# Gadersd/whisper-burn

Hardware: NVIDIA H100
Metric: audio-seconds/sec (higher is better)
Workload: dtype f32 (fp16-exact weights, fp32 activations/accumulate)

## Files before the change

whisper-burn_b200/csrc/api.cu:

```cuda
#include <algorithm>
#include <cstring>
#include <map>
#include <memory>
#include <mutex>
#include <new>

#include "../host/beam.hpp"
#include "../host/repeat.hpp"
#include "session.h"

struct wb_model {
    wb::Model impl;
    std::mutex fwd_mu;
    std::unique_ptr<wb::Session> fwd;
    wb::Session& forward_session(int64_t n_windows, int64_t text_len) {
        if (!fwd || fwd->max_windows < n_windows || fwd->t_max < text_len) {
            fwd.reset();
            fwd.reset(new wb::Session(&impl, std::max<int64_t>(n_windows, 1), 1, std::max<int64_t>(text_len, 2), WB_KV_F32));
        }
        return *fwd;
    }
    ~wb_model() { fwd.reset(); }
};
struct wb_session {
// ... 351 lines not shown
        if (!S.encoded) wb::fail(WB_ERR_STATE, "get_mel: nothing encoded");
        WB_REQUIRE(window >= 0 && window < S.n_windows, "get_mel: window out of range");
        const int Tm = S.win_Tm[(size_t)window];
        WB_REQUIRE(capacity >= (int64_t)Tm * wb::N_MELS, "get_mel: capacity too small");
        std::vector<float> rows((size_t)Tm * wb::N_MELS);
        WB_CUDA(cudaMemcpy(rows.data(), S.mel_rows.p + ((int64_t)window * S.TmS + 1) * wb::N_MELS,
                           rows.size() * sizeof(float), cudaMemcpyDeviceToHost));
        for (int t = 0; t < Tm; ++t)
            for (int c = 0; c < wb::N_MELS; ++c) mel_out[(int64_t)c * Tm + t] = rows[(size_t)t * wb::N_MELS + c];
        *n_ctx_out = Tm;
    });
}

int wb_session_get_encoder_output(wb_session* s, int64_t window, float* out, int64_t capacity, int64_t* n_ctx_out) {
    return guarded([&] {
        WB_REQUIRE(s && out && n_ctx_out, "get_encoder_output: null pointer");
        wb::Session& S = *s->impl;
        if (!S.encoded) wb::fail(WB_ERR_STATE, "get_encoder_output: nothing encoded");
        WB_REQUIRE(window >= 0 && window < S.n_windows, "get_encoder_output: window out of range");
        const int d = S.m->dims.n_audio_state;
        const int T = S.win_T[(size_t)window];
        WB_REQUIRE(capacity >= (int64_t)T * d, "get_encoder_output: capacity too small");
        WB_CUDA(cudaMemcpy(out, S.xa.p + S.win_row_off[(size_t)window] * d, (size_t)T * d * sizeof(float),
                           cudaMemcpyDeviceToHost));
        *n_ctx_out = T;
    });
}

int wb_session_begin(wb_session* s, const int64_t* prompt, int64_t prompt_len) {
    return guarded([&] {
        WB_REQUIRE(s && prompt, "begin: null pointer");
        WB_REQUIRE(prompt_len >= 1, "begin: prompt length out of range");
        s->impl->begin(std::vector<std::vector<int64_t>>((size_t)s->impl->n_windows, std::vector<int64_t>(prompt, prompt + prompt_len)));
    });
}

int wb_session_step(wb_session* s, int64_t n_rows, const int32_t* window_of_row, const int32_t* parent_row,
                    const int64_t* token, int apply_special_mask, const uint8_t* is_special, int k,
                    int64_t* topk_ids_out, float* topk_logprob_out) {
    return guarded([&] {
        WB_REQUIRE(s && window_of_row && parent_row && token && topk_ids_out && topk_logprob_out, "step: null pointer");
        if (is_special) s->impl->set_special(is_special);
        WB_REQUIRE(!apply_special_mask || s->impl->have_special, "step: special mask requested but no is_special bitmap given");
        s->impl->step_beams(n_rows, window_of_row, parent_row, token, apply_special_mask, k, topk_ids_out, topk_logprob_out);
    });
}

int wb_transcribe_windows(wb_session* s, const float* const* waves, const int64_t* lens, int64_t n_windows,
                          int beam_size, int max_depth, const wb_special_ids* ids, const uint8_t* is_special,
                          int64_t* tokens_out, int64_t capacity, int64_t* lens_out) {
    return guarded([&] {
        WB_REQUIRE(s && waves && lens && ids && tokens_out && lens_out, "transcribe: null pointer");
        wb::Session& S = *s->impl;
        const auto prompts = wb::window_prompts(S, n_windows, beam_size, max_depth, *ids, is_special);
        copy_tokens_out(wb::transcribe_windows(S, prompts, beam_size, max_depth, ids->eot, is_special, capacity,
                                               [&] { S.encode_waveforms_host(waves, lens, n_windows); }),
                        tokens_out, capacity, lens_out);
    });
}

int wb_transcribe_windows_prev(wb_session* s, const float* const* waves, const int64_t* lens, int64_t n_windows,
                               const int64_t* prev_tokens, const int64_t* prev_lens, int64_t startofprev, int beam_size,
                               int max_depth, const wb_special_ids* ids, const uint8_t* is_special, int64_t* tokens_out,
                               int64_t capacity, int64_t* lens_out) {
    return guarded([&] {
        WB_REQUIRE(s && waves && lens && prev_lens && ids && tokens_out && lens_out, "transcribe_windows_prev: null pointer");
// ... 263 lines not shown
```

whisper-burn_b200/csrc/session.cu:

```cuda
#include <algorithm>
#include <cmath>
#include <cstdio>
#include <cstdlib>
#include <cstring>

#include "session.h"

namespace wb {

int window_mel_frames(int n_audio_ctx, int window_mode) {
    WB_REQUIRE(window_mode == WB_WINDOWS_REFERENCE || window_mode == WB_WINDOWS_NATIVE,
               "window_mode must be WB_WINDOWS_REFERENCE or WB_WINDOWS_NATIVE");
    return window_mode == WB_WINDOWS_NATIVE ? 2 * n_audio_ctx : n_audio_ctx;
}

int64_t window_samples(int n_audio_ctx, int window_mode) {
    return wb_max_waveform_samples(window_mel_frames(n_audio_ctx, window_mode) - MEL_PADDING);
}

Session::Session(Model* model, int64_t max_w, int64_t max_b, int64_t max_text_len, int kv, int mode) : m(model) {
    if (!m || !m->finalized) fail(WB_ERR_STATE, "session: model not finalized");
    const wb_dims& D = m->dims;
    WB_REQUIRE(max_w >= 1 && max_b >= 1 && max_w * max_b <= 4096, "session: bad max_windows / max_beams");
    WB_REQUIRE(max_text_len >= 2 && max_text_len <= D.n_text_ctx, "session: max_text_len must be in [2, n_text_ctx]");
// ... 54 lines not shown
    is_special.alloc(V);
    {
        ckv_tmp.alloc(Mcap * 2 * d);
        cudaDeviceProp prop;
        WB_CUDA(cudaGetDeviceProperties(&prop, m->device));
        n_sm = prop.multiProcessorCount;
        const int n_logit_ctas = 2 * prop.multiProcessorCount;
        part_o.alloc((size_t)Rmax * H * 16 * 64); part_m.alloc((size_t)Rmax * H * 16); part_l.alloc((size_t)Rmax * H * 16);
        datt.alloc((size_t)Rmax * d); steps_done.alloc(128); dec_bar.alloc(4);
        WB_CUDA(cudaMemsetAsync(dec_bar.p, 0, 4 * sizeof(unsigned int), st));
        {
            const bool h16 = m->fp16_exact;
            auto wp = [&](const LinearW& w) -> const void* { return h16 ? (const void*)w.w16 : (const void*)w.w32; };
            std::vector<DecLayer> lay((size_t)L);
            for (int l = 0; l < L; ++l) {
                const DecBlockW& B = m->dec[(size_t)l];
                DecLayer& y = lay[(size_t)l];
                y.ln1_g = B.attn_ln.g; y.ln1_b = B.attn_ln.b; y.ln1_eps = B.attn_ln.eps;
                y.ln2_g = B.cross_ln.g; y.ln2_b = B.cross_ln.b; y.ln2_eps = B.cross_ln.eps;
                y.ln3_g = B.mlp_ln.g; y.ln3_b = B.mlp_ln.b; y.ln3_eps = B.mlp_ln.eps;
                y.Wqkv = wp(B.qkv); y.Wo = wp(B.out); y.Wcq = wp(B.cq); y.Wco = wp(B.cout); y.W1 = wp(B.mlp1); y.W2 = wp(B.mlp2);
                y.bqkv = B.qkv.b; y.bo = B.out.b; y.bcq = B.cq.b; y.bco = B.cout.b; y.b1 = B.mlp1.b; y.b2 = B.mlp2.b;
            }
            dec_layers.alloc((size_t)L);
            WB_CUDA(cudaMemcpy(dec_layers.p, lay.data(), lay.size() * sizeof(DecLayer), cudaMemcpyHostToDevice));
        }
        dec5_build_tables(*m, n_sm, d5);
        ypart.alloc((size_t)4 * Rmax * d);
        lg_m.alloc((size_t)n_logit_ctas * Rmax); lg_s.alloc((size_t)n_logit_ctas * Rmax);
        lg_v.alloc((size_t)n_logit_ctas * Rmax * DEC_KC); lg_i.alloc((size_t)n_logit_ctas * Rmax * DEC_KC);
    }
    h_parent = pinned<int>(Rmax); h_window = pinned<int>(Rmax); h_token = pinned<int>(Rmax);
    h_topk_id = pinned<int>((size_t)Rmax * DEC_KC);
    WB_CUDA(cudaMemsetAsync(is_special.p, 0, V, st));

    DecArgs& a = dec_base;
    a.Rmax = Rmax; a.d = D.n_text_state; a.H = H; a.L = L; a.V = V; a.t_max = t_max; a.Mcap = Mcap;
    a.eps_outside = m->ln_eps_outside; a.qk_scale = (float)std::pow((double)D.n_text_state / (double)H, -0.25);
    a.layers = dec_layers.p; a.tok_emb = m->tok_emb32; a.pos_emb = m->dec_pos;
    a.E = m->fp16_exact ? (const void*)m->tok_emb16 : (const void*)m->tok_emb32;
    a.E_tiled = m->tok_emb16_tiled;
    a.lnf_g = m->dec_ln.g; a.lnf_b = m->dec_ln.b; a.lnf_eps = m->dec_ln.eps;
    a.x = dx.p; a.q = dq.p; a.att = datt.p; a.hid = dhid.p;
    a.ypart = ypart.p; a.lgbuf = logits.p; a.att_pl = att_pl.p; a.hid_pl = hid_pl.p;
    a.kv_half = kv == WB_KV_F16 ? 1 : 0;
    if (a.kv_half) { a.kc = kc16.p; a.vc = vc16.p; a.ckv = ckv16.p; } else { a.kc = kc.p; a.vc = vc.p; a.ckv = ckv.p; }
    a.row_window = row_window.p; a.win_row_off = d_win_row_off.p; a.win_T = d_win_T.p;
    a.part_o = part_o.p; a.part_m = part_m.p; a.part_l = part_l.p;
    a.tokens = tokens.p; a.token_lp = token_lp.p; a.cur_tok = cur_tok.p; a.lengths = lengths.p; a.finished = finished.p;
    a.eot_logit = eot_logit.p; a.topk_id = topk_id.p; a.topk_lp = topk_lp.p;
    a.lg_m = lg_m.p; a.lg_s = lg_s.p; a.lg_v = lg_v.p; a.lg_i = lg_i.p;
    a.pos = pos.p; a.n_unfinished = n_unfinished.p; a.steps_done = steps_done.p; a.bar = dec_bar.p;
    WB_CUDA(cudaStreamSynchronize(st));
}

Session::~Session() {
    if (st) cudaStreamSynchronize(st);
    for (auto& e : ev)
        if (e) cudaEventDestroy(e);
    if (st) cudaStreamDestroy(st);
}

static void set_geometry(Session& s, const std::vector<int>& Tm, const std::vector<int>& F) {
    s.n_windows = (int)Tm.size();
    s.win_Tm = Tm;
    s.win_F = F;
    s.win_T.resize(Tm.size());
    s.win_row_off.resize(Tm.size());
    s.M_tot = 0;
    s.max_T = 0;
    s.max_Tm = 0;
    for (size_t w = 0; w < Tm.size(); ++w) {
        s.win_T[w] = (Tm[w] - 1) / 2 + 1;
        s.win_row_off[w] = s.M_tot;
        s.M_tot += s.win_T[w];
        s.max_T = std::max(s.max_T, s.win_T[w]);
        s.max_Tm = std::max(s.max_Tm, Tm[w]);
    }
    const int d = s.m->dims.n_audio_state;
    std::vector<GemmGroup> g1(Tm.size()), g2(Tm.size());
    std::vector<AttnWindow> aw(Tm.size());
    for (size_t w = 0; w < Tm.size(); ++w) {
        g1[w] = GemmGroup{(int64_t)w * s.TmS * N_MELS, ((int64_t)w * s.TmS + 1) * d, Tm[w]};
        g2[w] = GemmGroup{(int64_t)w * s.TmS * d, s.win_row_off[w] * d, s.win_T[w]};
        aw[w] = AttnWindow{s.win_row_off[w], s.win_T[w]};
    }
    WB_CUDA(cudaMemcpyAsync(s.d_g1.p, g1.data(), g1.size() * sizeof(GemmGroup), cudaMemcpyHostToDevice, s.st));
    WB_CUDA(cudaMemcpyAsync(s.d_g2.p, g2.data(), g2.size() * sizeof(GemmGroup), cudaMemcpyHostToDevice, s.st));
    WB_CUDA(cudaMemcpyAsync(s.d_awin.p, aw.data(), aw.size() * sizeof(AttnWindow), cudaMemcpyHostToDevice, s.st));
    WB_CUDA(cudaMemcpyAsync(s.d_win_row_off.p, s.win_row_off.data(), Tm.size() * sizeof(int64_t),
                            cudaMemcpyHostToDevice, s.st));
    WB_CUDA(cudaMemcpyAsync(s.d_win_T.p, s.win_T.data(), Tm.size() * sizeof(int), cudaMemcpyHostToDevice, s.st));
    WB_CUDA(cudaStreamSynchronize(s.st));
}

void Session::encode_from_device_wave(const float* wave_dev, const int64_t* offsets, const int64_t* lens, int64_t n) {
    WB_REQUIRE(n >= 1 && n <= max_windows, "encode: n_windows out of range for this session");
    std::vector<LogMelWindow> lw((size_t)n);
    std::vector<int> Tm((size_t)n), kept((size_t)n);
    int max_frames = 0;
    for (int64_t w = 0; w < n; ++w) {
        WB_REQUIRE(lens[w] >= N_FFT, "prep_audio: waveform shorter than n_fft (audio.rs:292)");
        WB_REQUIRE(lens[w] < (int64_t)1 << 30, "prep_audio: waveform too long");
        const int F = (int)(lens[w] / HOP);
        const int keep = std::min(F, mel_limit - MEL_PADDING);
        Tm[(size_t)w] = keep + MEL_PADDING;
        kept[(size_t)w] = keep;
        lw[(size_t)w] = LogMelWindow{offsets[w], (int)lens[w], F, keep, (int)w, ((int64_t)w * TmS + 1) * N_MELS};
        max_frames = std::max(max_frames, F);
    }
    WB_CUDA(cudaMemcpyAsync(d_lmwin.p, lw.data(), lw.size() * sizeof(LogMelWindow), cudaMemcpyHostToDevice, st));
    set_geometry(*this, Tm, kept);
    WB_CUDA(cudaEventRecord(ev[0], st));
    WB_CUDA(cudaMemsetAsync(mel_rows.p, 0, (size_t)n * TmS * N_MELS * sizeof(float), st));
    launch_logmel(*m, wave_dev, d_lmwin.p, (int)n, max_frames, mel_rows.p, max_slots.p, (int)n, st);
    WB_CUDA(cudaEventRecord(ev[1], st));
    run_encoder();
    WB_CUDA(cudaEventRecord(ev[2], st));
}

void Session::encode_waveforms_host(const float* const* waves, const int64_t* lens, int64_t n) {
    WB_REQUIRE(n >= 1 && n <= max_windows, "encode: n_windows out of range for this session");
    std::vector<int64_t> offs((size_t)n);
    int64_t total = 0;
    for (int64_t w = 0; w < n; ++w) {
        WB_REQUIRE(waves[w] != nullptr && lens[w] >= 0, "encode: null waveform");
        offs[(size_t)w] = total;
        total += (lens[w] + 3) / 4 * 4;
    }
    wave.ensure((size_t)total);
    for (int64_t w = 0; w < n; ++w)
        WB_CUDA(cudaMemcpyAsync(wave.p + offs[(size_t)w], waves[w], (size_t)lens[w] * sizeof(float),
                                cudaMemcpyHostToDevice, st));
    encode_from_device_wave(wave.p, offs.data(), lens, n);
}

void Session::encode_mels_host(const float* mel, int64_t n, int64_t n_mels, int64_t n_ctx) {
    const wb_dims& D = m->dims;
    WB_REQUIRE(n_mels == D.n_mels, "Audio mel spectrum size must be n_mels (mod.rs:231-235)");
    WB_REQUIRE(n_ctx >= 1 && n_ctx <= mel_limit, "Audio length cannot exceed the session's mel frame limit: n_audio_ctx, "
                                                 "2 * n_audio_ctx in native windowing (mod.rs:236-241)");
    WB_REQUIRE(n >= 1 && n <= max_windows, "encode: n_windows out of range for this session");
    std::vector<int> Tm((size_t)n, (int)n_ctx);
    set_geometry(*this, Tm, Tm);
    DevBuf<float> tmp;
// ... 106 lines not shown
        p = GemmParams{};
        p.A = hid.p; p.lda = 4 * d; p.B = B.mlp2.w32; p.C = x.p; p.ldc = d; p.N = d; p.K = 4 * d;
        p.bias = B.mlp2.b; p.residual = x.p; p.max_rows = M;
        launch_gemm(p, st);
    }
    launch_layernorm(x.p, xa.p, nullptr, nullptr, m->ln_post, M, d, m->ln_eps_outside, st);
}

void Session::run_cross_kv() {
    const wb_dims& D = m->dims;
    const int d = D.n_text_state;
    const float qk_scale = (float)std::pow((double)d / (double)D.n_text_head, -0.25);
    for (int l = 0; l < D.n_text_layer; ++l) {
        const DecBlockW& B = m->dec[(size_t)l];
        if (use_tc) {
            GemmF16Params p;
            p.A_hi = xa_h.p; p.A_lo = xa_l.p; p.lda = d; p.B = B.ckv.w16; p.C = ckv_tmp.p; p.ldc = 2 * d;
            p.N = 2 * d; p.K = d; p.bias = B.ckv.b; p.scale = qk_scale; p.scale_cols = d; p.max_rows = (int)M_tot;
            GemmF16Plan& pl = *enc_plans[(size_t)2 + 4 * D.n_audio_layer + l];
            if (!pl.matches(p.max_rows, 1)) pl.build(p, 0, (int)M_tot);
            pl.launch(st);
        } else {
            GemmParams p;
            p.A = xa.p; p.lda = d; p.B = B.ckv.w32; p.C = ckv_tmp.p; p.ldc = 2 * d;
            p.N = 2 * d; p.K = d; p.bias = B.ckv.b; p.scale = qk_scale; p.scale_cols = d; p.max_rows = (int)M_tot;
            launch_gemm(p, st);
        }
        void* dst = kv_dtype == WB_KV_F16 ? (void*)(ckv16.p + (size_t)l * Mcap * 2 * d) : (void*)(ckv.p + (size_t)l * Mcap * 2 * d);
        launch_ckv_relayout(ckv_tmp.p, dst, kv_dtype == WB_KV_F16, d_win_row_off.p, d_win_T.p, n_windows, M_tot, d, st);
    }
}

void Session::set_special(const uint8_t* sp) {
    if (sp) {
        WB_CUDA(cudaMemcpyAsync(is_special.p, sp, (size_t)m->dims.n_vocab, cudaMemcpyHostToDevice, st));
        WB_CUDA(cudaStreamSynchronize(st));
        have_special = true;
    }
}

void Session::seat_rows(int rows, int per_window, const std::vector<std::vector<int64_t>>& prompts, int max_depth) {
    if (!encoded) fail(WB_ERR_STATE, "session: decode before encode");
    WB_REQUIRE(rows <= Rmax && (int64_t)prompts.size() * per_window >= rows, "decode: rows out of range");
    const int V = m->dims.n_vocab;
    std::vector<int> tk((size_t)rows * t_max, 0), rw((size_t)rows), len((size_t)rows), lim((size_t)rows);
    for (int r = 0; r < rows; ++r) {
        const std::vector<int64_t>& pr = prompts[(size_t)(r / per_window)];
        WB_REQUIRE(!pr.empty() && (int64_t)pr.size() <= t_max, "decode: prompt length out of range");
        rw[(size_t)r] = r / per_window;
        len[(size_t)r] = (int)pr.size();
        lim[(size_t)r] = (int)pr.size() + max_depth;
        for (size_t i = 0; i < pr.size(); ++i) {
            WB_REQUIRE(pr[i] >= 0 && pr[i] < V, "decode: prompt token out of range");
            tk[(size_t)r * t_max + i] = (int)pr[i];
        }
    }
    WB_CUDA(cudaMemcpyAsync(tokens.p, tk.data(), tk.size() * sizeof(int), cudaMemcpyHostToDevice, st));
    WB_CUDA(cudaMemcpyAsync(row_window.p, rw.data(), rw.size() * sizeof(int), cudaMemcpyHostToDevice, st));
    WB_CUDA(cudaMemsetAsync(finished.p, 0, sizeof(int) * Rmax, st));
    WB_CUDA(cudaMemsetAsync(pos.p, 0, sizeof(int), st));
    WB_CUDA(cudaMemcpyAsync(lengths.p, len.data(), len.size() * sizeof(int), cudaMemcpyHostToDevice, st));
    WB_CUDA(cudaMemcpyAsync(lengths.p + Rmax, lim.data(), lim.size() * sizeof(int), cudaMemcpyHostToDevice, st));
    R = rows;
    anc_identity = true;
    anc_cur = 0;
    host_pos = 0;
}

void Session::feed_positions(int n, float* logits_out) {
    const size_t V = (size_t)m->dims.n_vocab;
    const StepLogits out = logits_out ? StepLogits::topk_and_raw : StepLogits::none;
    for (int p = 0; p < n; ++p, ++host_pos) {
        WB_CUDA(cudaMemcpy2DAsync(cur_tok.p, sizeof(int), tokens.p + p, t_max * sizeof(int), sizeof(int), R, cudaMemcpyDeviceToDevice, st));
        launch_decoder(DecodeLaunch::cached_step(R, host_pos, out, MASK_NONE, 1));
        if (logits_out)
            WB_CUDA(cudaMemcpy2DAsync(logits_out + p * V, n * V * sizeof(float), logits.p, V * sizeof(float), V * sizeof(float), R,
                                      cudaMemcpyDeviceToHost, st));
    }
}

static std::pair<int, int> prompt_range(const std::vector<std::vector<int64_t>>& prompts) {
    int lo = INT_MAX, hi = 0;
    for (const auto& pr : prompts) { lo = std::min(lo, (int)pr.size()); hi = std::max(hi, (int)pr.size()); }
    return {lo, hi};
}

void Session::begin(const std::vector<std::vector<int64_t>>& prompts, bool prefill, int max_depth) {
    WB_REQUIRE((int64_t)prompts.size() == n_windows, "begin: one prompt per encoded window");
    for (const auto& pr : prompts) WB_REQUIRE(!pr.empty() && (int64_t)pr.size() < t_max, "begin: prompt length out of range");
    seat_rows(n_windows, 1, prompts, max_depth);
    if (prefill) feed_positions(prompt_range(prompts).first - 1, nullptr);
    WB_CUDA(cudaStreamSynchronize(st));
}

void Session::teacher_forced_logits(const int64_t* toks, int64_t n_rows, int64_t seq_len, float* logits_out) {
    WB_REQUIRE(n_rows >= 1 && seq_len >= 1, "forward_decoder: empty input");
    std::vector<std::vector<int64_t>> rows((size_t)n_rows);
    for (int64_t r = 0; r < n_rows; ++r) rows[(size_t)r].assign(toks + r * seq_len, toks + (r + 1) * seq_len);
    seat_rows((int)n_rows, 1, rows);
    feed_positions((int)seq_len, logits_out);
    WB_CUDA(cudaStreamSynchronize(st));
}

bool Session::launch_decoder(const DecodeLaunch& l) {
    DecArgs a = dec_base;
    a.R = l.rows;
    a.lg_slices = std::max(1, std::min(16, n_sm / std::max(1, l.rows)));
    a.n_splits = std::max(1, std::min(16, n_sm / std::max(1, l.rows * a.H)));
    a.anc = anc_identity ? nullptr : (anc_cur == 0 ? anc0.p : anc1.p);
    a.use_cur_tok = l.use_cur_tok; a.pos0 = l.pos0; a.n_steps = l.n_steps; a.logits_from = l.logits_from;
    a.is_special = have_special ? is_special.p : nullptr; a.mask_mode = l.mask_mode;
    a.k = l.k; a.greedy = l.greedy; a.eot = l.eot; a.loop_rules = l.loop_rules; a.max_depth = l.max_depth;
    a.logits_out = l.raw_logits ? logits.p : nullptr;
    if (getenv("WB200_TRACE")) {
        dec_trace.ensure(1 << 16);
        WB_CUDA(cudaMemsetAsync(dec_trace.p, 0, sizeof(unsigned long long) * (1 << 16), st));
        a.trace = dec_trace.p;
        a.trace_cap = 1 << 16;
    }
    WB_CUDA(cudaMemsetAsync(dec_bar.p, 0, 4 * sizeof(unsigned int), st));
    const bool h16 = m->fp16_exact;
    auto allowed = [&](int n) { return only_decoder == 0 || only_decoder == n; };
    int groups = 0;
    last_groups = 1;
    if (l.beam > 1) {
// ... 63 lines not shown
    }
    {
        int* cur = anc_cur == 0 ? anc0.p : anc1.p;
        int* nxt = anc_cur == 0 ? anc1.p : anc0.p;
        R = (int)n_rows;
        launch_dec_reorder(cur, nxt, parent.p, pos.p, R, t_max, st);
        anc_cur ^= 1;
    }
    launch_decoder(DecodeLaunch::cached_step(R, host_pos, StepLogits::topk, apply_mask ? MASK_ALWAYS : MASK_NONE, k));
    ++host_pos;
    WB_CUDA(cudaMemcpyAsync(h_topk_id.get(), topk_id.p, sizeof(int) * n_rows * k, cudaMemcpyDeviceToHost, st));
    WB_CUDA(cudaMemcpyAsync(topk_lp_out, topk_lp.p, sizeof(float) * n_rows * k, cudaMemcpyDeviceToHost, st));
    WB_CUDA(cudaStreamSynchronize(st));
    for (int64_t i = 0; i < n_rows * k; ++i) topk_ids_out[i] = h_topk_id[i];
}

void Session::last_topk(int64_t n_rows, int64_t k, int64_t* ids_out, float* lp_out) {
    if (last_decoder == 0) fail(WB_ERR_STATE, "last_topk: no decoder launch yet");
    WB_REQUIRE(k == last_k, "last_topk: k differs from the last launch's k");
    WB_REQUIRE(n_rows >= 1 && n_rows <= last_rows, "last_topk: n_rows exceeds the last launch's rows");
    std::vector<int> ids((size_t)(n_rows * k));
    WB_CUDA(cudaStreamSynchronize(st));
    WB_CUDA(cudaMemcpy(ids.data(), topk_id.p, ids.size() * sizeof(int), cudaMemcpyDeviceToHost));
    WB_CUDA(cudaMemcpy(lp_out, topk_lp.p, ids.size() * sizeof(float), cudaMemcpyDeviceToHost));
    for (size_t i = 0; i < ids.size(); ++i) ids_out[i] = ids[i];
}

void Session::greedy_decode(const std::vector<std::vector<int64_t>>& prompts, int max_depth, int64_t eot,
                            std::vector<std::vector<int64_t>>& out, std::vector<std::vector<float>>& out_lp, bool loop_rules) {
    const auto [min_lp, max_lp] = prompt_range(prompts);
    WB_REQUIRE(max_lp + max_depth <= t_max, "greedy: prompt + max_depth exceeds the session's max_text_len");
    begin(prompts, false, max_depth);
    if (max_depth > 0) launch_decoder(DecodeLaunch::greedy_search(R, min_lp, max_lp, max_depth, (int)eot, loop_rules));
    std::vector<int> tk((size_t)R * t_max), len((size_t)R);
    std::vector<float> lp((size_t)R * t_max);
    int sdv[128] = {0};
    WB_CUDA(cudaMemcpyAsync(tk.data(), tokens.p, tk.size() * sizeof(int), cudaMemcpyDeviceToHost, st));
    WB_CUDA(cudaMemcpyAsync(lp.data(), token_lp.p, lp.size() * sizeof(float), cudaMemcpyDeviceToHost, st));
    WB_CUDA(cudaMemcpyAsync(len.data(), lengths.p, len.size() * sizeof(int), cudaMemcpyDeviceToHost, st));
    if (max_depth > 0) WB_CUDA(cudaMemcpyAsync(sdv, steps_done.p, sizeof(int) * std::min(last_groups, 128), cudaMemcpyDeviceToHost, st));
    WB_CUDA(cudaStreamSynchronize(st));
    int sd = 0;
    for (int g = 0; g < std::min(last_groups, 128); ++g) sd = std::max(sd, sdv[g]);
    last_steps = max_depth > 0 ? sd - (min_lp - 1) : 0;
    host_pos = min_lp - 1 + (int)last_steps;
    out.assign((size_t)R, {});
    out_lp.assign((size_t)R, {});
    for (int r = 0; r < R; ++r) {
        const int64_t prompt_len = (int64_t)prompts[(size_t)r].size();
        for (int i = 0; i < len[(size_t)r]; ++i) {
            out[(size_t)r].push_back(tk[(size_t)r * t_max + i]);
            out_lp[(size_t)r].push_back(i < prompt_len ? 0.0f : lp[(size_t)r * t_max + i]);
        }
        if (loop_rules && max_depth > 0 && len[(size_t)r] <= prompt_len) out_lp[(size_t)r].back() = std::nanf("");
        if (loop_rules && out[(size_t)r].back() != eot) {
            out[(size_t)r].push_back(eot);
            out_lp[(size_t)r].push_back(std::nanf(""));
        }
    }
}

bool Session::beam_decode(const std::vector<std::vector<int64_t>>& prompts, int beam_size, int max_depth, int64_t eot,
                          std::vector<std::vector<int64_t>>& out, std::vector<std::vector<float>>& out_lp,
                          std::vector<NBest>& nbest) {
    namespace fx = beamfx;
    const auto [min_lp, max_lp] = prompt_range(prompts);
    WB_REQUIRE(min_lp >= 1 && max_lp + max_depth <= t_max, "beam: prompt + max_depth exceeds the session's max_text_len");
    const int B = beam_size, W = n_windows, Rb = W * B;
    if (B < 2 || B > fx::MAX_BEAM || max_depth < 1 || Rb > Rmax) return false;
    seat_rows(Rb, B, prompts, max_depth);
    constexpr int MN = fx::MAX_NODES;
    slot_live.ensure((size_t)Rmax);
// ... 71 lines not shown
```

whisper-burn_b200/csrc/session.h:

```cpp
#pragma once
#include <climits>
#include <functional>
#include <memory>
#include <vector>

#include "decoder.h"
#include "wb_internal.h"

namespace wb {

constexpr int MEL_PADDING = 10;

int window_mel_frames(int n_audio_ctx, int window_mode);
int64_t window_samples(int n_audio_ctx, int window_mode);

enum class StepLogits { none, topk, topk_and_raw };

struct DecodeLaunch {
    int rows = 0, pos0 = 0, n_steps = 1, logits_from = INT_MAX;
    bool use_cur_tok = false, raw_logits = false;
    int mask_mode = MASK_NONE, k = 1, eot = -1;
    bool greedy = false, loop_rules = false;
    int beam = 0, max_depth = 0;

// ... 34 lines not shown
};
struct AlignWs {
    DevBuf<AlignSeq> seqs;
    DevBuf<int64_t> out_off;
    DevBuf<int> heads, start, end;
    DevBuf<float> w, mat;
    DevBuf<double> stats;
};

struct PinnedFree { void operator()(void* p) const { cudaFreeHost(p); } };
template <typename T> using Pinned = std::unique_ptr<T[], PinnedFree>;
template <typename T> Pinned<T> pinned(size_t n) { void* p = nullptr; WB_CUDA(cudaMallocHost(&p, n * sizeof(T))); return Pinned<T>((T*)p); }

struct Session {
    Model* m = nullptr;
    cudaStream_t st = nullptr;
    int max_windows = 0, max_beams = 0, t_max = 0, kv_dtype = WB_KV_F32;
    int window_mode = WB_WINDOWS_REFERENCE;
    int search = WB_SEARCH_BEAM;
    int64_t startofprev = -1;
    int mel_limit = 0;
    int Rmax = 0;
    int TmS = 0;
    int Tcap = 0;
    int64_t Mcap = 0;

    int n_windows = 0;
    std::vector<int> win_Tm, win_T;
    std::vector<int> win_F;
    std::vector<int64_t> win_row_off;
    int64_t M_tot = 0;
    int max_T = 0, max_Tm = 0;
    bool encoded = false;

    DevBuf<LogMelWindow> d_lmwin;
    DevBuf<GemmGroup> d_g1, d_g2;
    DevBuf<AttnWindow> d_awin;
    DevBuf<int64_t> d_win_row_off;
    DevBuf<int> d_win_T;
    DevBuf<float> wave;
    ResampleBufs rs;
    DevBuf<int> max_slots;
    DevBuf<float> mel_rows, x, xa;
    DevBuf<float> h1, xn, att, qkv, hid;
    DevBuf<__half> mel_h, mel_l, h1_h, h1_l, xn_h, xn_l, qkv_h, qkv_l, att_h, att_l, hid_h, hid_l, xa_h, xa_l;
    std::vector<std::unique_ptr<GemmF16Plan>> enc_plans;
    bool use_tc = true;
    void run_encoder_f16();
    void run_encoder_f32();
    DevBuf<float> ckv;
    DevBuf<float> ckv_tmp;
    DevBuf<float> kc, vc;
    DevBuf<__half> kc16, vc16, ckv16;
    DevBuf<float> dx, dq, dhid, logits;
    Dec5Tables d5;
    DevBuf<uint4> att_pl, hid_pl;
    DevBuf<float> part_o, part_m, part_l;
    DevBuf<int> tokens, lengths, cur_tok, finished, row_window, anc0, anc1, parent, pos, n_unfinished, topk_id;
    DevBuf<float> topk_lp;
    DevBuf<float> token_lp;
    DevBuf<float> eot_logit;
    DevBuf<uint8_t> is_special;
    bool have_special = false;
    int anc_cur = 0;
    bool anc_identity = true;
    int R = 0;
    int host_pos = 0;
    Pinned<int> h_parent, h_window, h_token, h_topk_id;
    cudaEvent_t ev[6] = {};
    float last_ms[4] = {0, 0, 0, 0};
    int64_t last_steps = 0;
    std::vector<std::vector<float>> last_logprobs;
    bool have_logprobs = false;
    std::vector<NBest> last_nbest;
    bool have_nbest = false;
    int last_groups = 1;
    int last_decoder = 0;
    int last_rows = 0, last_k = 0;
    int only_decoder = 0;
    int n_sm = 0;
    DevBuf<DecLayer> dec_layers;
    Dec6Pack d6;
    DevBuf<unsigned int> dec_bar;
    DevBuf<int> steps_done;
    DevBuf<float> datt;
    DevBuf<unsigned long long> dec_trace;
    DecArgs dec_base;
    bool launch_decoder(const DecodeLaunch& l);
    DevBuf<int> slot_live, bm_seq, bm_cnt, bm_win, bm_out, bm_out_len;
    DevBuf<float> bm_seq_lp, bm_out_lp;
    DevBuf<beamfx::Head> bm_head;
    DevBuf<float> ypart, lg_m, lg_s, lg_v;
    DevBuf<int> lg_i;
    void profile_decode(const int64_t* prompt, int64_t prompt_len, int n_steps, float* logits_ms, float* step_ms);

    Session(Model* model, int64_t max_windows, int64_t max_beams, int64_t max_text_len, int kv_dtype,
            int window_mode = WB_WINDOWS_REFERENCE);
    ~Session();
    Session(const Session&) = delete;
    Session& operator=(const Session&) = delete;

// ... 69 lines not shown
```

whisper-burn_b200/transcribe.py:

```python
from __future__ import annotations

import base64
import ctypes as C
import gzip
from typing import List, Optional, Sequence, Tuple

import numpy as np

from . import ffi
from .model import Whisper


WINDOW_MODES = {"reference": ffi.WB_WINDOWS_REFERENCE, "native": ffi.WB_WINDOWS_NATIVE}
SEARCH_RULES = {"beam": ffi.WB_SEARCH_BEAM, "greedy_loop": ffi.WB_SEARCH_GREEDY_LOOP}


def window_samples(n_audio_ctx: int, mode: str = "reference") -> int:
    n = int(ffi.lib().wb_window_samples(n_audio_ctx, WINDOW_MODES[mode]))
    if n < 0:
        raise ValueError(f"window_samples: n_audio_ctx {n_audio_ctx} out of range")
    return n


def _special(is_special: Optional[np.ndarray]):
# ... 61 lines not shown
    def get_encoder_output(self, window: int) -> np.ndarray:
        d = self.whisper.config.n_audio_state
        cap = d * ((self.max_mel_frames - 1) // 2 + 1)
        buf = np.empty(cap, dtype=np.float32)
        n = C.c_int64(0)
        ffi.check(ffi.lib().wb_session_get_encoder_output(self._h, window, ffi.fptr(buf), cap, C.byref(n)))
        return buf[:d * n.value].reshape(n.value, d).copy()

    def begin(self, prompt: Sequence[int]) -> None:
        p = np.asarray(prompt, dtype=np.int64)
        ffi.check(ffi.lib().wb_session_begin(self._h, ffi.i64ptr(p), len(p)))

    def step(self, window_of_row, parent_row, token, apply_special_mask: bool, is_special: Optional[np.ndarray], k: int):
        w = np.asarray(window_of_row, dtype=np.int32)
        pr = np.asarray(parent_row, dtype=np.int32)
        tk = np.asarray(token, dtype=np.int64)
        n = len(w)
        ids = np.empty((n, k), dtype=np.int64)
        lps = np.empty((n, k), dtype=np.float32)
        ffi.check(ffi.lib().wb_session_step(self._h, n, ffi.i32ptr(w), ffi.i32ptr(pr), ffi.i64ptr(tk),
                                           1 if apply_special_mask else 0, _special(is_special), k, ffi.i64ptr(ids),
                                           ffi.fptr(lps)))
        return ids, lps

    def transcribe_windows(self, waves: Sequence[np.ndarray], special, is_special: np.ndarray, beam_size: int = 5,
                           max_depth: int = 100) -> List[List[int]]:
        ws, ptrs, lens = _host_waves(waves)
        cap = 4 + max_depth + 1
        out = np.zeros((len(ws), cap), dtype=np.int64)
        out_len = np.zeros(len(ws), dtype=np.int64)
        ffi.check(ffi.lib().wb_transcribe_windows(self._h, ptrs, ffi.i64ptr(lens), len(ws), beam_size, max_depth,
                                                 C.byref(_special_ids(special)), _special(is_special), ffi.i64ptr(out), cap,
                                                 ffi.i64ptr(out_len)))
        return [[int(t) for t in out[i, :out_len[i]]] for i in range(len(ws))]

    def transcribe_windows_prev(self, waves: Sequence[np.ndarray], prev: Sequence[Sequence[int]], special,
                                is_special: Optional[np.ndarray], beam_size: int = 5, max_depth: int = 100,
                                startofprev: Optional[int] = None) -> List[List[int]]:
        ws, ptrs, lens = _host_waves(waves)
        if len(prev) != len(ws):
            raise ValueError(f"transcribe_windows_prev: {len(ws)} windows but {len(prev)} previous-id lists")
        prev_lens = np.asarray([len(p) for p in prev], dtype=np.int64)
        prev_toks = np.ascontiguousarray(np.concatenate([np.asarray(p, dtype=np.int64) for p in prev] + [np.zeros(1, np.int64)]))
        cap = max([4] + [len(p) + 5 for p in prev if len(p)]) + max_depth + 1
        out = np.zeros((len(ws), cap), dtype=np.int64)
        out_len = np.zeros(len(ws), dtype=np.int64)
        sop = special.startofprev if startofprev is None else startofprev
        ffi.check(ffi.lib().wb_transcribe_windows_prev(self._h, ptrs, ffi.i64ptr(lens), len(ws), ffi.i64ptr(prev_toks),
                                                      ffi.i64ptr(prev_lens), sop, beam_size, max_depth,
                                                      C.byref(_special_ids(special)),
                                                      _special(is_special), ffi.i64ptr(out), cap, ffi.i64ptr(out_len)))
        return [[int(t) for t in out[i, :out_len[i]]] for i in range(len(ws))]

    def transcribe_windows_dev(self, wave_dev_ptr: int, offsets, lens, special, is_special: np.ndarray,
                               beam_size: int = 5, max_depth: int = 100) -> List[List[int]]:
        offs = np.asarray(offsets, dtype=np.int64)
        ln = np.asarray(lens, dtype=np.int64)
        cap = 4 + max_depth + 1
        out = np.zeros((len(ln), cap), dtype=np.int64)
        out_len = np.zeros(len(ln), dtype=np.int64)
        ffi.check(ffi.lib().wb_transcribe_windows_dev(self._h, C.c_void_p(wave_dev_ptr), ffi.i64ptr(offs), ffi.i64ptr(ln),
                                                     len(ln), beam_size, max_depth, C.byref(_special_ids(special)),
                                                     _special(is_special), ffi.i64ptr(out), cap, ffi.i64ptr(out_len)))
        return [[int(t) for t in out[i, :out_len[i]]] for i in range(len(ln))]

    def waveform_to_tokens(self, waveform: np.ndarray, special, is_special: np.ndarray, sample_rate: int = 16000,
                           beam_size: int = 5, max_depth: int = 100) -> List[int]:
        w = np.ascontiguousarray(waveform, dtype=np.float32)
        cap = (len(w) // 1000 + 2) * (10 + max_depth + 1) + 16
        out = np.zeros(cap, dtype=np.int64)
        n = C.c_int64(0)
        ffi.check(ffi.lib().wb_waveform_to_tokens(self._h, ffi.fptr(w), len(w), sample_rate, beam_size, max_depth,
                                                 C.byref(_special_ids(special)), _special(is_special), ffi.i64ptr(out), cap,
                                                 C.byref(n)))
        return [int(t) for t in out[:n.value]]

    def waveforms_to_tokens(self, waveforms: Sequence[np.ndarray], special, is_special: np.ndarray, sample_rate: int = 16000,
                            beam_size: int = 5, max_depth: int = 100) -> List[List[int]]:
        ws, ptrs, lens = _host_waves(waveforms)
        cap = (max(len(w) for w in ws) // 1000 + 2) * (10 + max_depth + 1) + 16
        out = np.zeros((len(ws), cap), dtype=np.int64)
        n = np.zeros(len(ws), dtype=np.int64)
        ffi.check(ffi.lib().wb_waveforms_to_tokens(self._h, ptrs, ffi.i64ptr(lens), len(ws), sample_rate, beam_size, max_depth,
                                                  C.byref(_special_ids(special)), _special(is_special), ffi.i64ptr(out), cap,
                                                  ffi.i64ptr(n)))
        return [[int(t) for t in out[i, :n[i]]] for i in range(len(ws))]

    def waveforms_to_tokens_resampled(self, waveforms: Sequence[np.ndarray], sample_rates: Sequence[int], special,
                                      is_special: np.ndarray, beam_size: int = 5, max_depth: int = 100) -> List[List[int]]:
        from .audio import _frames, resampled_length
        ws = [_frames(w) for w in waveforms]
        if len(sample_rates) != len(ws):
            raise ValueError("one sample rate per waveform")
        ptrs = (ffi._F * len(ws))(*[ffi.fptr(w) for w in ws])
        frames = np.asarray([w.shape[0] for w in ws], dtype=np.int64)
        channels = np.asarray([w.shape[1] for w in ws], dtype=np.int64)
        rates = np.asarray(sample_rates, dtype=np.int64)
        n16 = max(max(resampled_length(int(n), int(r)) for n, r in zip(frames, rates)), 0)
        cap = (n16 // 1000 + 2) * (10 + max_depth + 1) + 16
        out = np.zeros((len(ws), cap), dtype=np.int64)
        n = np.zeros(len(ws), dtype=np.int64)
        ffi.check(ffi.lib().wb_waveforms_to_tokens_resampled(self._h, ptrs, ffi.i64ptr(frames), ffi.i64ptr(channels),
                                                            ffi.i64ptr(rates), len(ws), beam_size, max_depth,
                                                            C.byref(_special_ids(special)), _special(is_special),
                                                            ffi.i64ptr(out), cap, ffi.i64ptr(n)))
        return [[int(t) for t in out[i, :n[i]]] for i in range(len(ws))]

    def last_logprobs(self, index: int) -> np.ndarray:
        n = C.c_int64(0)
        ffi.check(ffi.lib().wb_session_last_logprobs(self._h, index, None, 0, C.byref(n)))
        out = np.empty(n.value, dtype=np.float32)
        ffi.check(ffi.lib().wb_session_last_logprobs(self._h, index, ffi.fptr(out), n.value, C.byref(n)))
        return out

    def last_nbest(self, index: int):
        n = C.c_int64(0)
        ffi.check(ffi.lib().wb_session_last_nbest(self._h, index, 0, 0, None, None, None, None, None, C.byref(n)))
        lens = np.zeros(max(n.value, 1), dtype=np.int64)
        ffi.check(ffi.lib().wb_session_last_nbest(self._h, index, n.value, 0, None, None, ffi.i64ptr(lens), None, None,
                                                  C.byref(n)))
        cap = max(int(lens[:n.value].max(initial=0)), 1)
        ids = np.zeros((max(n.value, 1), cap), dtype=np.int64)
        lps = np.zeros((max(n.value, 1), cap), dtype=np.float32)
        scores = np.zeros(max(n.value, 1), dtype=np.float64)
        fin = np.zeros(max(n.value, 1), dtype=np.int32)
        ffi.check(ffi.lib().wb_session_last_nbest(self._h, index, n.value, cap, ffi.i64ptr(ids), ffi.fptr(lps), ffi.i64ptr(lens),
                                                  scores.ctypes.data_as(C.POINTER(C.c_double)), ffi.i32ptr(fin), C.byref(n)))
        return [([int(t) for t in ids[r, :lens[r]]], lps[r, :lens[r]].copy(), float(scores[r]), bool(fin[r]))
                for r in range(n.value)]

    def score_tokens(self, seqs: Sequence[Sequence[int]], windows: Sequence[int], apply_special_mask: bool = False,
                     is_special: Optional[np.ndarray] = None):
        lens = np.asarray([len(s) for s in seqs], dtype=np.int64)
        toks = np.ascontiguousarray(np.concatenate([np.asarray(s, dtype=np.int64) for s in seqs]) if len(seqs)
                                    else np.zeros(0, dtype=np.int64), dtype=np.int64)
        win = np.ascontiguousarray(windows, dtype=np.int32)
        if len(win) != len(lens):
            raise ValueError(f"score_tokens: {len(lens)} sequences but {len(win)} windows")
        lp = np.empty(max(len(toks), 1), dtype=np.float32)
# ... 133 lines not shown
```

Baseline: 2576.

## Cut host-side syncs and copies across encode, seating and readback

Caches the log-mel window table, the window geometry and the special-token mask on the host, so identical re-uploads and their stream syncs are skipped. Seats prompt rows from a pinned staging buffer guarded by an event, and drops the unconditional stream sync in begin (the C API keeps one). Greedy readback now lands in pinned host buffers, and the Python wrappers convert token arrays with tolist(). The aim is less per-call host latency and fewer pageable copies. The cost is extra state that could go stale, and an event wait on the staging buffer.

```diff
diff --git a/whisper-burn_b200/csrc/api.cu b/whisper-burn_b200/csrc/api.cu
--- a/whisper-burn_b200/csrc/api.cu
+++ b/whisper-burn_b200/csrc/api.cu
@@ -407,6 +407,7 @@
         WB_REQUIRE(s && prompt, "begin: null pointer");
         WB_REQUIRE(prompt_len >= 1, "begin: prompt length out of range");
         s->impl->begin(std::vector<std::vector<int64_t>>((size_t)s->impl->n_windows, std::vector<int64_t>(prompt, prompt + prompt_len)));
+        WB_CUDA(cudaStreamSynchronize(s->impl->st));
     });
 }
 
diff --git a/whisper-burn_b200/csrc/session.cu b/whisper-burn_b200/csrc/session.cu
--- a/whisper-burn_b200/csrc/session.cu
+++ b/whisper-burn_b200/csrc/session.cu
@@ -110,6 +110,9 @@
     }
     h_parent = pinned<int>(Rmax); h_window = pinned<int>(Rmax); h_token = pinned<int>(Rmax);
     h_topk_id = pinned<int>((size_t)Rmax * DEC_KC);
+    h_seat = pinned<int>((size_t)Rmax * t_max + 3 * (size_t)Rmax);
+    h_out_tok = pinned<int>((size_t)Rmax * t_max); h_out_lp = pinned<float>((size_t)Rmax * t_max); h_out_len = pinned<int>((size_t)Rmax + 128);
+    WB_CUDA(cudaEventCreateWithFlags(&seat_done, cudaEventDisableTiming));
     WB_CUDA(cudaMemsetAsync(is_special.p, 0, V, st));
 
     DecArgs& a = dec_base;
@@ -136,10 +139,13 @@
     if (st) cudaStreamSynchronize(st);
     for (auto& e : ev)
         if (e) cudaEventDestroy(e);
+    if (seat_done) cudaEventDestroy(seat_done);
     if (st) cudaStreamDestroy(st);
 }
 
-static void set_geometry(Session& s, const std::vector<int>& Tm, const std::vector<int>& F) {
+static bool set_geometry(Session& s, const std::vector<int>& Tm, const std::vector<int>& F) {
+    if (s.geometry_set && Tm == s.win_Tm && F == s.win_F) return false;
+    s.geometry_set = false;
     s.n_windows = (int)Tm.size();
     s.win_Tm = Tm;
     s.win_F = F;
@@ -170,6 +176,8 @@
                             cudaMemcpyHostToDevice, s.st));
     WB_CUDA(cudaMemcpyAsync(s.d_win_T.p, s.win_T.data(), Tm.size() * sizeof(int), cudaMemcpyHostToDevice, s.st));
     WB_CUDA(cudaStreamSynchronize(s.st));
+    s.geometry_set = true;
+    return true;
 }
 
 void Session::encode_from_device_wave(const float* wave_dev, const int64_t* offsets, const int64_t* lens, int64_t n) {
@@ -187,8 +195,12 @@
         lw[(size_t)w] = LogMelWindow{offsets[w], (int)lens[w], F, keep, (int)w, ((int64_t)w * TmS + 1) * N_MELS};
         max_frames = std::max(max_frames, F);
     }
-    WB_CUDA(cudaMemcpyAsync(d_lmwin.p, lw.data(), lw.size() * sizeof(LogMelWindow), cudaMemcpyHostToDevice, st));
-    set_geometry(*this, Tm, kept);
+    const bool new_lw = lw.size() != lmwin_host.size() || std::memcmp(lw.data(), lmwin_host.data(), lw.size() * sizeof(LogMelWindow)) != 0;
+    if (new_lw) {
+        lmwin_host = lw;
+        WB_CUDA(cudaMemcpyAsync(d_lmwin.p, lmwin_host.data(), lw.size() * sizeof(LogMelWindow), cudaMemcpyHostToDevice, st));
+    }
+    if (!set_geometry(*this, Tm, kept) && new_lw) WB_CUDA(cudaStreamSynchronize(st));
     WB_CUDA(cudaEventRecord(ev[0], st));
     WB_CUDA(cudaMemsetAsync(mel_rows.p, 0, (size_t)n * TmS * N_MELS * sizeof(float), st));
     launch_logmel(*m, wave_dev, d_lmwin.p, (int)n, max_frames, mel_rows.p, max_slots.p, (int)n, st);
@@ -361,35 +373,44 @@
 }
 
 void Session::set_special(const uint8_t* sp) {
-    if (sp) {
-        WB_CUDA(cudaMemcpyAsync(is_special.p, sp, (size_t)m->dims.n_vocab, cudaMemcpyHostToDevice, st));
-        WB_CUDA(cudaStreamSynchronize(st));
-        have_special = true;
-    }
+    if (!sp) return;
+    const size_t V = (size_t)m->dims.n_vocab;
+    if (have_special && std::memcmp(special_host.data(), sp, V) == 0) return;
+    have_special = false;
+    special_host.assign(sp, sp + V);
+    WB_CUDA(cudaMemcpyAsync(is_special.p, special_host.data(), V, cudaMemcpyHostToDevice, st));
+    WB_CUDA(cudaStreamSynchronize(st));
+    have_special = true;
 }
 
 void Session::seat_rows(int rows, int per_window, const std::vector<std::vector<int64_t>>& prompts, int max_depth) {
     if (!encoded) fail(WB_ERR_STATE, "session: decode before encode");
     WB_REQUIRE(rows <= Rmax && (int64_t)prompts.size() * per_window >= rows, "decode: rows out of range");
     const int V = m->dims.n_vocab;
-    std::vector<int> tk((size_t)rows * t_max, 0), rw((size_t)rows), len((size_t)rows), lim((size_t)rows);
     for (int r = 0; r < rows; ++r) {
         const std::vector<int64_t>& pr = prompts[(size_t)(r / per_window)];
         WB_REQUIRE(!pr.empty() && (int64_t)pr.size() <= t_max, "decode: prompt length out of range");
-        rw[(size_t)r] = r / per_window;
-        len[(size_t)r] = (int)pr.size();
-        lim[(size_t)r] = (int)pr.size() + max_depth;
-        for (size_t i = 0; i < pr.size(); ++i) {
-            WB_REQUIRE(pr[i] >= 0 && pr[i] < V, "decode: prompt token out of range");
-            tk[(size_t)r * t_max + i] = (int)pr[i];
-        }
-    }
-    WB_CUDA(cudaMemcpyAsync(tokens.p, tk.data(), tk.size() * sizeof(int), cudaMemcpyHostToDevice, st));
-    WB_CUDA(cudaMemcpyAsync(row_window.p, rw.data(), rw.size() * sizeof(int), cudaMemcpyHostToDevice, st));
+        for (int64_t t : pr) WB_REQUIRE(t >= 0 && t < V, "decode: prompt token out of range");
+    }
+    WB_CUDA(cudaEventSynchronize(seat_done));
+    int* tk = h_seat.get();
+    int* rw = tk + (size_t)rows * t_max;
+    int* len = rw + rows;
+    std::memset(tk, 0, (size_t)rows * t_max * sizeof(int));
+    for (int r = 0; r < rows; ++r) {
+        const std::vector<int64_t>& pr = prompts[(size_t)(r / per_window)];
+        rw[r] = r / per_window;
+        len[r] = (int)pr.size();
+        len[rows + r] = (int)pr.size() + max_depth;
+        for (size_t i = 0; i < pr.size(); ++i) tk[(size_t)r * t_max + i] = (int)pr[i];
+    }
+    WB_CUDA(cudaMemcpyAsync(tokens.p, tk, (size_t)rows * t_max * sizeof(int), cudaMemcpyHostToDevice, st));
+    WB_CUDA(cudaMemcpyAsync(row_window.p, rw, rows * sizeof(int), cudaMemcpyHostToDevice, st));
     WB_CUDA(cudaMemsetAsync(finished.p, 0, sizeof(int) * Rmax, st));
     WB_CUDA(cudaMemsetAsync(pos.p, 0, sizeof(int), st));
-    WB_CUDA(cudaMemcpyAsync(lengths.p, len.data(), len.size() * sizeof(int), cudaMemcpyHostToDevice, st));
-    WB_CUDA(cudaMemcpyAsync(lengths.p + Rmax, lim.data(), lim.size() * sizeof(int), cudaMemcpyHostToDevice, st));
+    WB_CUDA(cudaMemcpyAsync(lengths.p, len, rows * sizeof(int), cudaMemcpyHostToDevice, st));
+    WB_CUDA(cudaMemcpyAsync(lengths.p + Rmax, len + rows, rows * sizeof(int), cudaMemcpyHostToDevice, st));
+    WB_CUDA(cudaEventRecord(seat_done, st));
     R = rows;
     anc_identity = true;
     anc_cur = 0;
@@ -419,7 +440,6 @@
     for (const auto& pr : prompts) WB_REQUIRE(!pr.empty() && (int64_t)pr.size() < t_max, "begin: prompt length out of range");
     seat_rows(n_windows, 1, prompts, max_depth);
     if (prefill) feed_positions(prompt_range(prompts).first - 1, nullptr);
-    WB_CUDA(cudaStreamSynchronize(st));
 }
 
 void Session::teacher_forced_logits(const int64_t* toks, int64_t n_rows, int64_t seq_len, float* logits_out) {
@@ -549,12 +569,14 @@
     WB_REQUIRE(max_lp + max_depth <= t_max, "greedy: prompt + max_depth exceeds the session's max_text_len");
     begin(prompts, false, max_depth);
     if (max_depth > 0) launch_decoder(DecodeLaunch::greedy_search(R, min_lp, max_lp, max_depth, (int)eot, loop_rules));
-    std::vector<int> tk((size_t)R * t_max), len((size_t)R);
-    std::vector<float> lp((size_t)R * t_max);
-    int sdv[128] = {0};
-    WB_CUDA(cudaMemcpyAsync(tk.data(), tokens.p, tk.size() * sizeof(int), cudaMemcpyDeviceToHost, st));
-    WB_CUDA(cudaMemcpyAsync(lp.data(), token_lp.p, lp.size() * sizeof(float), cudaMemcpyDeviceToHost, st));
-    WB_CUDA(cudaMemcpyAsync(len.data(), lengths.p, len.size() * sizeof(int), cudaMemcpyDeviceToHost, st));
+    const int* tk = h_out_tok.get();
+    const float* lp = h_out_lp.get();
+    const int* len = h_out_len.get();
+    int* sdv = h_out_len.get() + Rmax;
+    std::fill(sdv, sdv + 128, 0);
+    WB_CUDA(cudaMemcpyAsync(h_out_tok.get(), tokens.p, (size_t)R * t_max * sizeof(int), cudaMemcpyDeviceToHost, st));
+    WB_CUDA(cudaMemcpyAsync(h_out_lp.get(), token_lp.p, (size_t)R * t_max * sizeof(float), cudaMemcpyDeviceToHost, st));
+    WB_CUDA(cudaMemcpyAsync(h_out_len.get(), lengths.p, R * sizeof(int), cudaMemcpyDeviceToHost, st));
     if (max_depth > 0) WB_CUDA(cudaMemcpyAsync(sdv, steps_done.p, sizeof(int) * std::min(last_groups, 128), cudaMemcpyDeviceToHost, st));
     WB_CUDA(cudaStreamSynchronize(st));
     int sd = 0;
diff --git a/whisper-burn_b200/csrc/session.h b/whisper-burn_b200/csrc/session.h
--- a/whisper-burn_b200/csrc/session.h
+++ b/whisper-burn_b200/csrc/session.h
@@ -90,6 +90,8 @@
     int64_t M_tot = 0;
     int max_T = 0, max_Tm = 0;
     bool encoded = false;
+    bool geometry_set = false;
+    std::vector<LogMelWindow> lmwin_host;
 
     DevBuf<LogMelWindow> d_lmwin;
     DevBuf<GemmGroup> d_g1, d_g2;
@@ -120,11 +122,15 @@
     DevBuf<float> eot_logit;
     DevBuf<uint8_t> is_special;
     bool have_special = false;
+    std::vector<uint8_t> special_host;
     int anc_cur = 0;
     bool anc_identity = true;
     int R = 0;
     int host_pos = 0;
     Pinned<int> h_parent, h_window, h_token, h_topk_id;
+    Pinned<int> h_seat, h_out_tok, h_out_len;
+    Pinned<float> h_out_lp;
+    cudaEvent_t seat_done = nullptr;
     cudaEvent_t ev[6] = {};
     float last_ms[4] = {0, 0, 0, 0};
     int64_t last_steps = 0;
diff --git a/whisper-burn_b200/transcribe.py b/whisper-burn_b200/transcribe.py
--- a/whisper-burn_b200/transcribe.py
+++ b/whisper-burn_b200/transcribe.py
@@ -117,7 +117,7 @@
         ffi.check(ffi.lib().wb_transcribe_windows(self._h, ptrs, ffi.i64ptr(lens), len(ws), beam_size, max_depth,
                                                  C.byref(_special_ids(special)), _special(is_special), ffi.i64ptr(out), cap,
                                                  ffi.i64ptr(out_len)))
-        return [[int(t) for t in out[i, :out_len[i]]] for i in range(len(ws))]
+        return [out[i, :out_len[i]].tolist() for i in range(len(ws))]
 
     def transcribe_windows_prev(self, waves: Sequence[np.ndarray], prev: Sequence[Sequence[int]], special,
                                 is_special: Optional[np.ndarray], beam_size: int = 5, max_depth: int = 100,
@@ -135,7 +135,7 @@
                                                       ffi.i64ptr(prev_lens), sop, beam_size, max_depth,
                                                       C.byref(_special_ids(special)),
                                                       _special(is_special), ffi.i64ptr(out), cap, ffi.i64ptr(out_len)))
-        return [[int(t) for t in out[i, :out_len[i]]] for i in range(len(ws))]
+        return [out[i, :out_len[i]].tolist() for i in range(len(ws))]
 
     def transcribe_windows_dev(self, wave_dev_ptr: int, offsets, lens, special, is_special: np.ndarray,
                                beam_size: int = 5, max_depth: int = 100) -> List[List[int]]:
@@ -147,7 +147,7 @@
         ffi.check(ffi.lib().wb_transcribe_windows_dev(self._h, C.c_void_p(wave_dev_ptr), ffi.i64ptr(offs), ffi.i64ptr(ln),
                                                      len(ln), beam_size, max_depth, C.byref(_special_ids(special)),
                                                      _special(is_special), ffi.i64ptr(out), cap, ffi.i64ptr(out_len)))
-        return [[int(t) for t in out[i, :out_len[i]]] for i in range(len(ln))]
+        return [out[i, :out_len[i]].tolist() for i in range(len(ln))]
 
     def waveform_to_tokens(self, waveform: np.ndarray, special, is_special: np.ndarray, sample_rate: int = 16000,
                            beam_size: int = 5, max_depth: int = 100) -> List[int]:
@@ -158,7 +158,7 @@
         ffi.check(ffi.lib().wb_waveform_to_tokens(self._h, ffi.fptr(w), len(w), sample_rate, beam_size, max_depth,
                                                  C.byref(_special_ids(special)), _special(is_special), ffi.i64ptr(out), cap,
                                                  C.byref(n)))
-        return [int(t) for t in out[:n.value]]
+        return out[:n.value].tolist()
 
     def waveforms_to_tokens(self, waveforms: Sequence[np.ndarray], special, is_special: np.ndarray, sample_rate: int = 16000,
                             beam_size: int = 5, max_depth: int = 100) -> List[List[int]]:
@@ -169,7 +169,7 @@
         ffi.check(ffi.lib().wb_waveforms_to_tokens(self._h, ptrs, ffi.i64ptr(lens), len(ws), sample_rate, beam_size, max_depth,
                                                   C.byref(_special_ids(special)), _special(is_special), ffi.i64ptr(out), cap,
                                                   ffi.i64ptr(n)))
-        return [[int(t) for t in out[i, :n[i]]] for i in range(len(ws))]
+        return [out[i, :n[i]].tolist() for i in range(len(ws))]
 
     def waveforms_to_tokens_resampled(self, waveforms: Sequence[np.ndarray], sample_rates: Sequence[int], special,
                                       is_special: np.ndarray, beam_size: int = 5, max_depth: int = 100) -> List[List[int]]:
@@ -189,7 +189,7 @@
                                                             ffi.i64ptr(rates), len(ws), beam_size, max_depth,
                                                             C.byref(_special_ids(special)), _special(is_special),
                                                             ffi.i64ptr(out), cap, ffi.i64ptr(n)))
-        return [[int(t) for t in out[i, :n[i]]] for i in range(len(ws))]
+        return [out[i, :n[i]].tolist() for i in range(len(ws))]
 
     def last_logprobs(self, index: int) -> np.ndarray:
         n = C.c_int64(0)
```

Result: no change. 2597 (median of 6 runs) (+0.8%).
